# rarimo/ultragroth

Measured on AMD Instinct MI355X. Metric: proofs/s, higher is better.
Workload: dtype u32x9 (29-bit limbs, 254-bit modular integers)

## Files before the change

### ultragroth_amd/csrc/internal.hpp

```cpp
#pragma once
#include <hip/hip_runtime.h>
#include <cstdint>
#include <cstddef>
#include <vector>
#include "ec.hpp"
#include "stream_timer.hpp"

namespace ug {

Fr fr_root_of_unity(int s);
void bitrev_copy(u32* out, const u32* in, int logn, hipStream_t stream);

struct NttFusion {
    const u32* in2 = nullptr; u32* work = nullptr; const u32* fin_a = nullptr; const u32* fin_b = nullptr;
    u64 in2_stride = 0, work_stride = 0, fin_a_stride = 0, fin_b_stride = 0;
};

struct NttPass {
    const u32* in; u32* out; const u32* tw; const u32* post; const u32* post_const; const u32* in2; const u32* fin_a; const u32* fin_b;
    int logn, s0, k, j, gather_bitrev, scatter_bitrev;
    u64 in_stride, out_stride, in2_stride, fin_a_stride, fin_b_stride;
};
constexpr int NTT_MAX_PASSES = 8;

struct NttPlan {
    int logn = -1;
    u32* tw_fwd = nullptr;
    u32* tw_inv = nullptr;
    u32* twist = nullptr;
    u32* ninv = nullptr;
    bool shoup = true;
    void init(int logn, hipStream_t stream);
    void release();
    void transform(u32* out, const u32* in, bool inverse, bool gather_bitrev, bool scatter_bitrev,
                   const u32* post, const u32* post_const, hipStream_t stream, LaunchTimer stats = LaunchTimer(),
                   const struct NttFusion* fuse = nullptr, int vectors = 1, u64 out_stride = 0, u64 in_stride = 0) const;
    int passes(NttPass* list, u32* out, const u32* in, bool inverse, bool gather_bitrev, bool scatter_bitrev,
               const u32* post, const u32* post_const, const struct NttFusion* fuse = nullptr, u64 out_stride = 0, u64 in_stride = 0) const;
    void launch(const NttPass* const* lists, int count, int p, hipStream_t stream, LaunchTimer stats = LaunchTimer(), int vectors = 1) const;
    ~NttPlan() { release(); }
};

uint64_t alloc_epoch();
void alloc_epoch_bump();
template <class T> void epoch_alloc(T*& p, size_t bytes) { alloc_epoch_bump(); if (p) hipFree(p); p = nullptr; UG_HIP(hipMalloc(&p, bytes ? bytes : 4)); }

struct BucketClasses {
    int q_log = 0;
    u32 r0 = 0, cnt = 1;
    u32 specials = 0;
    u32 sp_lo = 0, sp_hi = 0;
    bool on() const { return q_log > 0; }
};
constexpr u32 MSM_MAX_SPECIALS = 64;

struct DigitPlan {
    u64 n; int c, windows; u32 buckets, sentinel; int tables;
    u64 set_map, table_map;
    int q_log; u32 r0, cnt, specials, sp_lo, sp_hi, special_base;
    u32 vec_count, vec_magic; int vec_shift; u32 vec_sets; u64 vec_stride;
};

struct MsmGeometry {
    u64 n = 0;
    int c = 0;
    int windows = 0;
    u32 buckets = 0;
    bool tables = false;
    int stride = 1;
    BucketClasses cls;
    int vectors = 1;
    u64 vec_stride = 0;
    static MsmGeometry choose(u64 n, int force_c = 0);
    static MsmGeometry choose_tables(u64 n, int c, int stride = 1);
    static int table_window(u64 n);
    static int table_count(int c, int stride) { const int w = (255 + c - 1) / c; return (w + stride - 1) / stride; }
    void set_classes(const BucketClasses& k);
    void set_vectors(int v, u64 stride);
    u64 vector_count() const { return n / (u64)vectors; }
    int window_sets() const { return tables ? stride : windows; }
    int class_sets() const { return cls.on() ? (int)cls.cnt : 1; }
    int bucket_windows() const { return window_sets() * class_sets() * vectors; }
    u64 special_buckets() const { return cls.on() ? (u64)window_sets() * cls.specials : 0; }
    u64 total_buckets() const { return (u64)bucket_windows() * buckets + special_buckets(); }
    int result_points() const { return cls.on() ? 2 * bucket_windows() + (cls.specials ? window_sets() : 0) : bucket_windows(); }
    u64 expected_entries() const { return cls.on() ? ((n * (u64)windows) >> cls.q_log) * cls.cnt : n * (u64)windows; }
    DigitPlan digit_plan() const {
        DigitPlan d;
        d.n = n; d.c = c; d.windows = windows; d.buckets = buckets; d.sentinel = (u32)total_buckets(); d.tables = tables ? 1 : 0;
        d.set_map = 0; d.table_map = 0;
        if (tables)
            for (int w = 0; w < windows && w < 16; w++) { d.set_map |= (u64)(w % stride) << (4 * w); d.table_map |= (u64)(w / stride) << (4 * w); }
        d.q_log = cls.q_log; d.r0 = cls.r0; d.cnt = cls.on() ? cls.cnt : 1; d.specials = cls.on() ? cls.specials : 0;
        d.sp_lo = cls.sp_lo; d.sp_hi = cls.sp_hi; d.special_base = (u32)((u64)bucket_windows() * buckets);
        d.vec_count = (u32)vector_count(); d.vec_magic = 0; d.vec_shift = 0; d.vec_sets = (u32)window_sets(); d.vec_stride = vec_stride;
        if (vectors > 1) {
            int l = 0;
            while (((u64)1 << l) < (u64)d.vec_count) l++;
            d.vec_magic = (u32)((((u64)1 << 32) * (((u64)1 << l) - d.vec_count)) / d.vec_count + 1);
            d.vec_shift = l;
        }
        return d;
    }
};
constexpr int MSM_MAX_VECTORS = 16;
constexpr int TABLE_INDEX_BITS = 27;
constexpr int TABLE_MIN_C = 16, TABLE_MAX_C = 24;
double msm_model_cost(u64 n, int c, bool tables, int stride = 1);

struct HeavyBucket { u32 bucket, first_seg, last_seg, pad; };

int radix_plan(int bits, int* shift, int* bins_log);
void digit_pairs(const u32* scalars, const DigitPlan& plan, u32* keys, u32* vals, hipStream_t stream);
struct RadixSorter {
    u32* lookback = nullptr;
    u32* small = nullptr;
    u64 tiles_cap = 0;
    void reserve(u64 n_pairs, int ipt_min);
    void release();
    int sort(const u32* scalars, const MsmGeometry& geo, u32 sentinel, u64 n_pairs, int bits,
             u32* const buf_keys[2], u32* const buf_vals[2], u32* error_flag, hipStream_t stream, u32* n_valid_out = nullptr,
             bool* dropped_out = nullptr);
    ~RadixSorter() { release(); }
};

struct MsmSchedule {
    MsmGeometry geo;
    const u32* keys = nullptr;
    const u32* vals = nullptr;
    const u32* tkeys = nullptr;
    const u32* tvals = nullptr;
    u32* bucket_start = nullptr;
    u32* bucket_count = nullptr;
    u32* small_list = nullptr;
    int log_seg = 0;
    int log_seg_tail = 0;
    u32* heavy_list = nullptr;
    u32 heavy_cap = 0;
    u32* medium_list = nullptr;
    u32* heavy_offsets = nullptr;
    u32* meta = nullptr;
    u32 *keys_a = nullptr, *keys_b = nullptr, *vals_a = nullptr, *vals_b = nullptr;
    void* sort_tmp = nullptr; size_t sort_tmp_bytes = 0;
    RadixSorter sorter;
    u64 capacity_n = 0; u64 capacity_buckets = 0;
    void reserve(const MsmGeometry& g);
    void build(const u32* scalars_dev, const MsmGeometry& g, hipStream_t stream);
    void release();
    ~MsmSchedule() { release(); }
};

struct MsmWorkspace {
    u32* bucket_pts = nullptr;
    u32* chunk_pts = nullptr;
    u32* chunk_pts2 = nullptr;
    u32* slot_pts = nullptr;
    u32* task_pts = nullptr;
    size_t bucket_bytes = 0, chunk_bytes = 0, slot_bytes = 0, task_bytes = 0;
    void reserve(const MsmGeometry& g, bool g2, u64 n_segments, u32 n_heavy_tasks, int sets = 1);
    void release();
    ~MsmWorkspace() { release(); }
};

struct MsmPending {
    bool g2 = false;
    bool empty = true;
    int c = 0, window_sets = 0, class_sets = 1;
    int vectors = 1;
    BucketClasses cls;
    u32* host = nullptr;
};
constexpr int MSM_G2_PT_WORDS = 72;
constexpr size_t MSM_PENDING_WORDS = 128 * 72;
constexpr int MSM_QUEUE_DEPTH = 8;
constexpr int MSM_BATCH_WIDTH = 4;
struct MsmCall {
    struct Product { const u32* bases = nullptr; u64 n_bases = 0; int64_t delta = 0; u32* host = nullptr; };
    int count = 0;
    Product products[MSM_BATCH_WIDTH];
    int group = 0;
};
constexpr int MSM_PHASE_ALL = 0, MSM_PHASE_ACCUMULATE = 1, MSM_PHASE_TAIL = 2;
void msm_enqueue(bool g2, const MsmSchedule& s, MsmWorkspace& ws, const MsmCall& call, hipStream_t stream, LaunchTimer stats, MsmPending* pend,
                 int phase = MSM_PHASE_ALL);
void interleave_points_g1(u32* dst, const u32* src, u64 n, int members, int member, u64 slot0, hipStream_t stream);
G1XYZZ msm_collect_g1(const MsmPending& p, int vector = 0);
G2XYZZ msm_collect_g2(const MsmPending& p, int vector = 0);

void convert_points_g1(u32* pts, u64 n, hipStream_t stream);
void convert_points_g2(u32* pts, u64 n, hipStream_t stream);

void build_window_tables(bool g2, u32* pts, u64 n, int doublings, int tables, hipStream_t stream, u64 first = 0, u64 count = ~(u64)0);

void synth_points(bool g2, u32* out_dev, const u32* gen_record_host, u64 seed, u64 n, hipStream_t stream);

void check_points(bool g2, const u32* pts, u64 n, u64 index0, int level, unsigned long long* fault, hipStream_t stream);
void check_points_mask(bool g2, const u32* pts, u64 n, int level, uint8_t* status, hipStream_t stream);

struct CoefMatrix {
    u64 ncoefs = 0; u32 domain = 0; int logn = 0;
    u32* row_ptr = nullptr;
    u32* sig = nullptr;
    u32* val = nullptr;
    bool build(const uint8_t* raw44_dev, u64 ncoefs, u32 domain, u32 nvars, hipStream_t stream);
    void release();
    ~CoefMatrix() { release(); }
};

void coef_matvec(u32* a_br, u32* b_br, const CoefMatrix& m, const u32* wtns_dev, int mask, hipStream_t stream);
constexpr int MATVEC_VT = 4;
void coef_matvec_vectors(u32* a_br, u32* b_br, u64 out_stride, const CoefMatrix& m, const u32* wtns_dev, u64 wtns_stride, int vectors,
                         hipStream_t stream);
void fr_mul_pointwise(u32* out, const u32* x, const u32* y, u64 n, hipStream_t stream);
void fr_h_final(u32* h, const u32* a, const u32* b, const u32* c, u64 n, hipStream_t stream);
void fr_h_final_vectors(u32* h, u64 h_stride, const u32* a, const u32* b, const u32* c, u64 in_stride, u64 n, int vectors, hipStream_t stream);
void fr_from_mont256(u32* out, const u32* in, u64 n, hipStream_t stream);
void fr_to_mont256(u32* out, const u32* in, u64 n, hipStream_t stream);
void f_op_mont256(int which, int op, u32* out, const u32* a, const u32* b, u64 n, hipStream_t stream);
void gather_elements(u32* out, const u32* src, const u32* index_dev, u64 n, u64 src_n, hipStream_t stream);
void scatter_elements(u32* dst, const u32* index_dev, const u32* values_dev, u64 n, u64 dst_n, hipStream_t stream);
void lookup_table(u32* table_dev, const u32* freq_dev, u64 L, hipStream_t stream);
void apply_lookup(u32* dst, u32* last_scratch, const u32* w_idx, const u32* p_idx, u64 n, const u32* chunks, u64 n_chunks,
                  const u32* table, hipStream_t stream);
struct LookupVec { u64 n, n_chunks, L, w_off, p_off, c_off, f_off, r_off, t_off; };
void lookup_tables_vectors(u32* stage, const LookupVec* vec_dev, int vectors, u64 max_L, hipStream_t stream);
void apply_lookup_vectors(u32* dst, u64 stride, u32* last_scratch, const u32* stage, const LookupVec* vec_dev, int vectors, u64 max_n,
                          hipStream_t stream);


struct R1csDev {
    u32 rows = 0;
    const u32* row_ptr[3] = {nullptr, nullptr, nullptr};
    const u32* sig[3] = {nullptr, nullptr, nullptr};
    const u32* val[3] = {nullptr, nullptr, nullptr};
};
void r1cs_convert_coefs(u32* val, u64 n, hipStream_t stream);
void r1cs_check(const R1csDev& m, const u32* wtns, unsigned long long* words, uint8_t* mask, hipStream_t stream);
void r1cs_row_values(const R1csDev& m, const u32* wtns, u32 k, u32* out24, hipStream_t stream);
void r1cs_match(const R1csDev& m, const CoefMatrix& zk, u32 n_public, const u32* z, unsigned long long* word, hipStream_t stream);

}
```

### ultragroth_amd/csrc/msm.hip

```cpp
#ifdef UG_MEASURE
#include <hipcub/hipcub.hpp>
#endif
#include <algorithm>
#include <atomic>
#include <cstdlib>
#include <cstring>
#include <string>
#include <type_traits>
#include "dev_common.hpp"
#include "internal.hpp"
#include "segmap.hpp"

namespace ug {

namespace {

constexpr int LOG_SEG = 7;
constexpr u32 FIX_MAX = 32;
constexpr u32 MEDIUM_MAX = 4096;
constexpr u32 HEAVY_TASK = 1024;
constexpr int CHUNK = 32;

constexpr int ACC_BLOCK = 256;

// ... 345 lines not shown
    u32 nkey = cur, nval = tvals[tbase];
    int64_t nidx = (int64_t)(nval & IDX_MASK) + delta;
    bool nin = nidx >= 0 && (u64)nidx < n_slots;
    if (nin) Cfg::load_raw(raw, record(nval, nidx, 0));
    for (u32 k = 0; k < cnt; k++) {
        const u32 key = nkey, val = nval;
        const int64_t idx = nidx;
        const bool in = nin;
        const bool more = k + 1 < cnt;
        if (more) {
            nkey = tkeys[tbase + ((u64)(k + 1) << 6)];
            nval = tvals[tbase + ((u64)(k + 1) << 6)];
            nidx = (int64_t)(nval & IDX_MASK) + delta;
            nin = nidx >= 0 && (u64)nidx < n_slots;
        }
        if (key != cur) {
            flush(first_run && start_open, (size_t)2 * t, cur);
            cur = key;
            first_run = false;
        }
        StaticFor<0, K>::up([&](auto m) {
            F x, y;
            const bool valid = in && Cfg::decode_affine(raw, x, y);
            if (m + 1 < K) { if (in) Cfg::load_raw(raw, record(val, idx, m + 1)); }
            else if (more && nin) Cfg::load_raw(raw, record(nval, nidx, 0));
            if (valid && (val >> 31)) y = neg<1>(y);
            if (valid) acc[m] = xyzz_madd(acc[m], x, y);
        });
    }
    const bool end_open = hi < n_valid && keys[hi] == cur;
    if (first_run && start_open) flush(true, (size_t)2 * t, 0);
    else if (end_open) flush(true, (size_t)2 * t + 1, 0);
    else flush(false, 0, cur);
}

template <class Cfg>
__device__ __forceinline__ XYZZ<typename Cfg::F> load_piece(const u32* slot_pts, u32 first, u32 k) {
    size_t slot = k ? (size_t)2 * (first + k) : (size_t)2 * first + 1;
    return Cfg::from_words(slot_pts + slot * Cfg::PT_WORDS, 1);
}

template <class Cfg>
__global__ __launch_bounds__(128) void bucket_fixup_kernel(const u32* __restrict__ small_list, const u32* __restrict__ meta,
                                                           const u32* __restrict__ start, const u32* __restrict__ count, int log_a, int log_b,
                                                           const u32* __restrict__ slot_pts, u32* __restrict__ bucket_pts,
                                                           size_t slot_stride, size_t bucket_stride) {
    u32 t = blockIdx.x * blockDim.x + threadIdx.x;
    if (t >= meta[4]) return;
    slot_pts += blockIdx.y * slot_stride; bucket_pts += blockIdx.y * bucket_stride;
    typedef typename Cfg::F F;
    const u32 b = small_list[t];
    const u32 st = start[b];
    const SegMap map = SegMap::make(meta[1], log_a, log_b);
    const u32 first = map.seg_of(st), last = map.seg_of(st + count[b] - 1);
    const u32 pieces = last - first + 1;
    XYZZ<F> acc = load_piece<Cfg>(slot_pts, first, 0);
    for (u32 k = 1; k < pieces; k++) acc = xyzz_add(acc, load_piece<Cfg>(slot_pts, first, k));
    Cfg::to_words(bucket_pts + (size_t)b * Cfg::PT_WORDS, acc, 1);
}

template <class Cfg>
__device__ __forceinline__ XYZZ<typename Cfg::F> block_reduce(XYZZ<typename Cfg::F> acc, u32* lds) {
    const int tid = threadIdx.x, nth = Cfg::BLOCK;
    for (int stride = nth / 2; stride > 0; stride >>= 1) {
        if (tid >= stride && tid < 2 * stride) Cfg::to_words(lds + (tid - stride), acc, stride);
        __syncthreads();
        if (tid < stride) acc = xyzz_add(acc, Cfg::from_words(lds + tid, stride));
        __syncthreads();
    }
    return acc;
}

template <class Cfg>
__global__ __launch_bounds__(256) void medium_bucket_kernel(const HeavyBucket* mb, const u32* meta, u32 cap, const u32* slot_pts, u32* bucket_pts,
                                                            size_t slot_stride, size_t bucket_stride) {
    typedef typename Cfg::F F;
    slot_pts += blockIdx.y * slot_stride; bucket_pts += blockIdx.y * bucket_stride;
    const u32 lane = threadIdx.x & 63, n_waves = (gridDim.x * blockDim.x) >> 6;
    const u32 n_medium = meta[3] < cap ? meta[3] : cap;
    for (u32 wave = (blockIdx.x * blockDim.x + threadIdx.x) >> 6; wave < n_medium; wave += n_waves) {
        HeavyBucket h = mb[wave];
        u32 pieces = h.last_seg - h.first_seg + 1;
        XYZZ<F> acc = xyzz_inf<F>();
        for (u32 k = lane; k < pieces; k += 64) acc = xyzz_add(acc, load_piece<Cfg>(slot_pts, h.first_seg, k));
        u32 w[Cfg::PT_WORDS];
        for (int off = 32; off > 0; off >>= 1) {
            Cfg::to_words(w, acc, 1);
#pragma unroll
            for (int i = 0; i < Cfg::PT_WORDS; i++) w[i] = __shfl_xor(w[i], off, 64);
            acc = xyzz_add(acc, Cfg::from_words(w, 1));
        }
        if (lane == 0) Cfg::to_words(bucket_pts + (size_t)h.bucket * Cfg::PT_WORDS, acc, 1);
    }
}

__global__ __launch_bounds__(1024) void heavy_plan_kernel(const HeavyBucket* hb, u32 n_heavy_cap, u32* meta, u32* offsets) {
    __shared__ u32 part[1024];
    const u32 n = meta[0] < n_heavy_cap ? meta[0] : n_heavy_cap;
    const u32 per = (n + 1023) / 1024;
    u32 lo = threadIdx.x * per, hi = lo + per < n ? lo + per : n;
    u32 sum = 0;
    for (u32 i = lo; i < hi; i++) sum += (hb[i].last_seg - hb[i].first_seg + 1 + HEAVY_TASK - 1) / HEAVY_TASK;
    part[threadIdx.x] = sum;
    __syncthreads();
    if (threadIdx.x == 0) {
        u32 run = 0;
        for (int i = 0; i < 1024; i++) { u32 v = part[i]; part[i] = run; run += v; }
        meta[2] = run;
        offsets[n] = run;
    }
    __syncthreads();
    u32 run = part[threadIdx.x];
    for (u32 i = lo; i < hi; i++) {
        offsets[i] = run;
        run += (hb[i].last_seg - hb[i].first_seg + 1 + HEAVY_TASK - 1) / HEAVY_TASK;
    }
}

template <class Cfg>
__global__ __launch_bounds__(Cfg::BLOCK) void heavy_partial_kernel(const HeavyBucket* hb, const u32* offsets, const u32* meta, u32 cap,
                                                                   const u32* slot_pts, u32* task_pts, size_t slot_stride, size_t task_stride) {
    __shared__ u32 lds[Cfg::PT_WORDS * Cfg::BLOCK / 2];
    typedef typename Cfg::F F;
    slot_pts += blockIdx.y * slot_stride; task_pts += blockIdx.y * task_stride;
    const u32 task = blockIdx.x;
    const u32 n_heavy = meta[0] < cap ? meta[0] : cap;
    if (task >= meta[2]) return;
    u32 lo = 0, hi = n_heavy;
    while (hi - lo > 1) { u32 mid = (lo + hi) >> 1; if (offsets[mid] <= task) lo = mid; else hi = mid; }
    HeavyBucket h = hb[lo];
    u32 pieces = h.last_seg - h.first_seg + 1;
    u32 p0 = (task - offsets[lo]) * HEAVY_TASK, p1 = p0 + HEAVY_TASK < pieces ? p0 + HEAVY_TASK : pieces;
    XYZZ<F> acc = xyzz_inf<F>();
    for (u32 k = p0 + threadIdx.x; k < p1; k += Cfg::BLOCK) acc = xyzz_add(acc, load_piece<Cfg>(slot_pts, h.first_seg, k));
    acc = block_reduce<Cfg>(acc, lds);
    if (threadIdx.x == 0) Cfg::to_words(task_pts + (size_t)task * Cfg::PT_WORDS, acc, 1);
}

template <class Cfg>
__global__ __launch_bounds__(Cfg::BLOCK) void heavy_final_kernel(const HeavyBucket* hb, const u32* offsets, const u32* meta, u32 cap,
                                                                 const u32* task_pts, u32* bucket_pts, size_t task_stride, size_t bucket_stride) {
    __shared__ u32 lds[Cfg::PT_WORDS * Cfg::BLOCK / 2];
    typedef typename Cfg::F F;
    task_pts += blockIdx.y * task_stride; bucket_pts += blockIdx.y * bucket_stride;
    if (blockIdx.x >= (meta[0] < cap ? meta[0] : cap)) return;
    HeavyBucket h = hb[blockIdx.x];
    u32 t0 = offsets[blockIdx.x], t1 = offsets[blockIdx.x + 1];
    XYZZ<F> acc = xyzz_inf<F>();
    for (u32 k = t0 + threadIdx.x; k < t1; k += Cfg::BLOCK) acc = xyzz_add(acc, Cfg::from_words(task_pts + (size_t)k * Cfg::PT_WORDS, 1));
    acc = block_reduce<Cfg>(acc, lds);
    if (threadIdx.x == 0) Cfg::to_words(bucket_pts + (size_t)h.bucket * Cfg::PT_WORDS, acc, 1);
}

template <class Cfg>
__global__ __launch_bounds__(128) void bucket_chunk_reduce_kernel(const u32* buckets, const u32* count, u32 per_window, int chunk,
                                                                  u32 nchunks_total, int scalar_bits, u32* out, u32 windows, u32* out0,
                                                                  size_t product_buckets) {
    u32 t = blockIdx.x * blockDim.x + threadIdx.x;
    if (t >= nchunks_total) return;
    typedef typename Cfg::F F;
    u32 chunks_per_window = per_window / chunk;
    u32 w = t / chunks_per_window, j = t % chunks_per_window;
    const size_t b0 = (size_t)(w / windows) * product_buckets + (size_t)(w % windows) * per_window + (size_t)j * chunk;
    const size_t c0 = (size_t)(w % windows) * per_window + (size_t)j * chunk;
    const u32* base = buckets + b0 * Cfg::PT_WORDS;
    XYZZ<F> run = xyzz_inf<F>(), acc = xyzz_inf<F>();
    for (int k = chunk - 1; k >= 0; k--) {
        if (count[c0 + k]) run = xyzz_add(run, Cfg::from_words(base + (size_t)k * Cfg::PT_WORDS, 1));
        acc = xyzz_add(acc, run);
    }
    u32 off = j * (u32)chunk;
    if (off) acc = xyzz_add(acc, xyzz_mul_scalar(run, &off, scalar_bits));
    Cfg::to_words(out + (size_t)t * Cfg::PT_WORDS, acc, 1);
    if (out0) Cfg::to_words(out0 + (size_t)t * Cfg::PT_WORDS, run, 1);
}
template <class Cfg>
__global__ __launch_bounds__(64) void special_sum_kernel(const u32* bucket_pts, const u32* count, u32 special_base, u32 S, size_t bucket_stride,
                                                         u32* out, u32 window_sets) {
    typedef typename Cfg::F F;
    const u32 w = blockIdx.x, q = blockIdx.y, lane = threadIdx.x;
    XYZZ<F> x = xyzz_inf<F>();
    const u32 id = special_base + w * S + lane;
    if (lane < S && count[id]) x = Cfg::from_words(bucket_pts + (size_t)q * bucket_stride + (size_t)id * Cfg::PT_WORDS, 1);
    XYZZ<F> acc = xyzz_inf<F>();
    const u32 k = lane + 1;
    for (int i = 6; i >= 0; i--) {
        acc = xyzz_dbl(acc);
        if ((k >> i) & 1) acc = xyzz_add(acc, x);
    }
    u32 v[Cfg::PT_WORDS];
    for (int off = 32; off > 0; off >>= 1) {
        Cfg::to_words(v, acc, 1);
#pragma unroll
        for (int i = 0; i < Cfg::PT_WORDS; i++) v[i] = __shfl_xor(v[i], off, 64);
        acc = xyzz_add(acc, Cfg::from_words(v, 1));
    }
    if (lane == 0) Cfg::to_words(out + ((size_t)q * window_sets + w) * Cfg::PT_WORDS, acc, 1);
}
template <class Cfg>
__global__ __launch_bounds__(128) void ec_sum_groups_kernel(const u32* in, u32* out, u32 n_out, int group) {
    u32 t = blockIdx.x * blockDim.x + threadIdx.x;
    if (t >= n_out) return;
    typedef typename Cfg::F F;
    XYZZ<F> acc = Cfg::from_words(in + (size_t)t * group * Cfg::PT_WORDS, 1);
    for (int g = 1; g < group; g++) acc = xyzz_add(acc, Cfg::from_words(in + ((size_t)t * group + g) * Cfg::PT_WORDS, 1));
    Cfg::to_words(out + (size_t)t * Cfg::PT_WORDS, acc, 1);
}

template <class Cfg>
__global__ __launch_bounds__(256) void ec_sum_wave_kernel(const u32* in, u32* out, u32 n_out, int group) {
    typedef typename Cfg::F F;
    const u32 wave = (blockIdx.x * blockDim.x + threadIdx.x) >> 6, lane = threadIdx.x & 63;
    if (wave >= n_out) return;
    XYZZ<F> acc = xyzz_inf<F>();
    for (int g = (int)lane; g < group; g += 64) acc = xyzz_add(acc, Cfg::from_words(in + ((size_t)wave * group + g) * Cfg::PT_WORDS, 1));
    u32 w[Cfg::PT_WORDS];
    for (int off = 32; off > 0; off >>= 1) {
        Cfg::to_words(w, acc, 1);
#pragma unroll
        for (int i = 0; i < Cfg::PT_WORDS; i++) w[i] = __shfl_xor(w[i], off, 64);
        acc = xyzz_add(acc, Cfg::from_words(w, 1));
    }
    if (lane == 0) Cfg::to_words(out + (size_t)wave * Cfg::PT_WORDS, acc, 1);
}

__global__ void convert_coords_kernel(u32* pts, u64 n_coords_groups, int coords_per_point) {
    u64 i = (u64)blockIdx.x * blockDim.x + threadIdx.x;
    if (i >= n_coords_groups) return;
    u32* p = pts + i * 8 * coords_per_point;
    u32 o = 0;
    for (int k = 0; k < 8 * coords_per_point; k++) o |= p[k];
    if (o == 0) return;
    for (int k = 0; k < coords_per_point; k++) {
        u32 w[8];
        load8(w, p + 8 * k);
        Fq v = cond_sub_q(from_mont256<FqParams>(w));
        pack256(w, v);
        store8(p + 8 * k, w);
    }
}

__global__ void interleave_records_kernel(u32* __restrict__ dst, const u32* __restrict__ src, u64 n, int members, int member, u64 slot0) {
    const u64 g = (u64)blockIdx.x * blockDim.x + threadIdx.x;
    if (g >= n * 4) return;
    const u64 i = g >> 2, part = g & 3;
    reinterpret_cast<uint4*>(dst + ((slot0 + i) * (u64)members + (u64)member) * 16)[part] = reinterpret_cast<const uint4*>(src + i * 16)[part];
}

template <class Cfg, int K>
__global__ __launch_bounds__(128) void window_tables_kernel(u32* pts, u64 n_all, int c, int tables, u64 first, u64 end) {
    typedef typename Cfg::F F;
    const u64 i0 = first + ((u64)blockIdx.x * blockDim.x + threadIdx.x) * K;
    const u64 n = end;
    if (i0 >= n) return;
    F x[K], y[K];
    bool live[K];
    StaticFor<0, K>::up([&](auto k) { live[k] = i0 + k < n && Cfg::load_affine(pts + (i0 + k) * Cfg::AFF_WORDS, x[k], y[k]); });
    for (int j = 1; j < tables; j++) {
        XYZZ<F> p[K];
        StaticFor<0, K>::up([&](auto k) { p[k] = live[k] ? xyzz_dbl_affine(x[k], y[k]) : xyzz_inf<F>(); });
        for (int d = 1; d < c; d++)
            StaticFor<0, K>::up([&](auto k) { p[k] = xyzz_dbl(p[k]); });
        F pre[K];
        F run = field_one((F*)0);
        StaticFor<0, K>::up([&](auto k) {
            pre[k] = run;
            if (live[k]) run = mulk<8>(run, p[k].zzz);
        });
        F irun = inv(run);
        StaticFor<0, K>::down([&](auto k) {
            if (i0 + k >= n) return;
            u32* o = pts + ((u64)j * n_all + i0 + k) * Cfg::AFF_WORDS;
            if (live[k]) {
                F izzz = mulk<8>(irun, pre[k]);
                irun = mulk<8>(irun, p[k].zzz);
                F iz = mulk<8>(izzz, p[k].zz);
                F izz = sqrk<8>(iz);
                x[k] = canon(mulk<8>(p[k].x, izz));
                y[k] = canon(mulk<8>(p[k].y, izzz));
                Cfg::store_affine_packed(o, x[k], y[k]);
            } else {
                for (int w = 0; w < Cfg::AFF_WORDS; w++) o[w] = 0;
            }
        });
    }
}

template <class Cfg>
__global__ __launch_bounds__(128) void synth_points_kernel(const u32* table, u64 seed, u64 n, u32* out) {
    u64 i = (u64)blockIdx.x * blockDim.x + threadIdx.x;
    if (i >= n) return;
    typedef typename Cfg::F F;
    u64 k = seed + i;
    XYZZ<F> acc = xyzz_inf<F>();
    for (int j = 0; j < 64; j++) {
        if (!((k >> j) & 1)) continue;
        F x, y;
        Cfg::load_affine(table + (size_t)j * Cfg::AFF_WORDS, x, y);
        acc = xyzz_madd(acc, x, y);
    }
    u32* o = out + i * Cfg::AFF_WORDS;
    if (is_inf(acc)) { for (int w = 0; w < Cfg::AFF_WORDS; w++) o[w] = 0; return; }
    F ax, ay;
    xyzz_to_affine(ax, ay, acc);
    Cfg::store_affine_mont256(o, ax, ay);
}

int reduce_chunk(const MsmGeometry& g, int sets = 1, bool g2 = false) {
    static const int g2_log = getenv("UG_REDUCE_G2_LOG") ? atoi(getenv("UG_REDUCE_G2_LOG")) : 16;
    static const int g1_log = getenv("UG_REDUCE_G1_LOG") ? atoi(getenv("UG_REDUCE_G1_LOG")) : 0;
    const int g1_auto = (u64)sets * g.bucket_windows() * g.buckets < ((u64)1 << 21) ? 16 : 17;
    const u64 lanes = (u64)1 << (g2 ? g2_log : (g1_log ? g1_log : g1_auto));
    int chunk = g.buckets < (u32)CHUNK ? (int)g.buckets : CHUNK;
    while (chunk > 8 && (u64)sets * g.bucket_windows() * (g.buckets / chunk) < lanes) chunk >>= 1;
    return chunk;
}

template <class T> void dev_free(T*& p) { if (p) { alloc_epoch_bump(); hipFree(p); } p = nullptr; }
std::atomic<uint64_t> g_alloc_epoch{1};

}

uint64_t alloc_epoch() { return g_alloc_epoch.load(std::memory_order_acquire); }
void alloc_epoch_bump() { g_alloc_epoch.fetch_add(1, std::memory_order_acq_rel); }

namespace {
int segment_log(u64 total_entries) {
    static const int lanes_log = getenv("UG_SEG_LANES_LOG") ? atoi(getenv("UG_SEG_LANES_LOG")) : 20;
    int log_seg = 5;
    while (log_seg < LOG_SEG && (total_entries >> (log_seg + 1)) >= ((u64)1 << lanes_log)) log_seg++;
    return log_seg;
}
double msm_cost(u64 n, int c, bool tables, int stride = 1) {
    const int windows = (255 + c - 1) / c;
    const double entries = (double)windows * (double)n, buckets = (double)((u64)1 << (c - 1));
    const double sets = tables ? (double)stride : (double)windows;
    const double per_bucket = entries / (sets * buckets);
    const double over = per_bucket / (double)((u64)1 << segment_log((u64)entries)) - 1.0;
    return entries * (1.0 + (over > 0 ? 0.04 * over : 0.0)) + 4.0 * buckets * sets;
}
}

double msm_model_cost(u64 n, int c, bool tables, int stride) { return msm_cost(n, c, tables, stride); }

MsmGeometry MsmGeometry::choose(u64 n, int force_c) {
    MsmGeometry g;
    g.n = n;
    int c = force_c;
    if (!c) {
        static const int env_c = getenv("UG_MSM_C") ? atoi(getenv("UG_MSM_C")) : 0;
        c = env_c;
    }
    if (!c) {
        double best = 0;
        for (int k = 6; k <= 22; k++) {
            double cost = msm_cost(n, k, false);
            if (!c || cost < best) { best = cost; c = k; }
        }
    }
    if (c < 2) c = 2;
    if (c > 22) c = 22;
    g.c = c;
    g.windows = (255 + c - 1) / c;
    g.buckets = 1u << (c - 1);
    return g;
}

int MsmGeometry::table_window(u64 n) {
    if (const char* e = getenv("UG_TABLE_C")) {
        int v = atoi(e);
        if (v >= TABLE_MIN_C && v <= TABLE_MAX_C) return v;
    }
    int c = 0;
    double best = 0;
    for (int k = TABLE_MIN_C; k <= TABLE_MAX_C; k++) {
        double cost = msm_cost(n, k, true);
        if (!c || cost < best) { best = cost; c = k; }
    }
    return c;
}
MsmGeometry MsmGeometry::choose_tables(u64 n, int c, int stride) {
    if (c < TABLE_MIN_C || c > TABLE_MAX_C) throw std::invalid_argument("msm: table window width outside [16, 24]");
    MsmGeometry g;
    g.n = n; g.c = c; g.tables = true;
    g.windows = (255 + c - 1) / c;
    g.buckets = 1u << (c - 1);
    if (stride < 1 || stride > g.windows)
        throw std::invalid_argument("msm: table stride " + std::to_string(stride) + " outside [1, " + std::to_string(g.windows) + "]");
    g.stride = stride;
    return g;
}

void MsmGeometry::set_classes(const BucketClasses& k) {
    cls = BucketClasses();
    if (!k.on()) return;
    if (k.q_log > 8) throw std::invalid_argument("msm: more than 256 bucket classes");
    if (tables && stride > 1) throw std::invalid_argument("msm: bucket classes need one bucket set per product (table stride 1)");
    const u32 Q = 1u << k.q_log;
    if (k.cnt < 1 || k.r0 + k.cnt > Q) throw std::invalid_argument("msm: bucket residues outside [0, 2^q_log)");
    if (k.specials > MSM_MAX_SPECIALS) throw std::invalid_argument("msm: more than 64 special buckets");
    if (k.sp_lo > k.sp_hi || k.sp_hi > n) throw std::invalid_argument("msm: special-bucket scalar range outside the schedule");
    if (c - 1 < k.q_log + 3 || ((u64)1 << (c - 1)) < k.specials) throw std::invalid_argument("msm: window too narrow for this many bucket classes");
    cls = k;
    buckets = 1u << (c - 1 - k.q_log);
    if ((size_t)result_points() * 72 > MSM_PENDING_WORDS - 1) throw std::invalid_argument("msm: too many bucket sets for one result block");
}

static_assert(G2Cfg::PT_WORDS == MSM_G2_PT_WORDS, "internal.hpp: MSM_G2_PT_WORDS");
void MsmGeometry::set_vectors(int v, u64 stride) {
    vectors = 1; vec_stride = 0;
    if (v == 1) return;
    if (v < 1 || v > MSM_MAX_VECTORS) throw std::invalid_argument("msm: vectors outside [1, " + std::to_string(MSM_MAX_VECTORS) + "]");
    if (cls.on()) throw std::invalid_argument("msm: bucket classes cannot be combined with several scalar vectors");
    if (stride < n) throw std::invalid_argument("msm: vector stride below the scalars per vector");
    if (n == 0) throw std::invalid_argument("msm: several vectors of no scalars");
    const u64 total = n * (u64)v;
    if (total * (u64)windows > ((u64)1 << 30)) throw std::invalid_argument("msm: vectors * n * windows exceeds 2^30 entries");
    if ((u64)window_sets() * (u64)v * buckets >= ((u64)1 << 31)) throw std::invalid_argument("msm: more than 2^31 buckets over all vectors");
    if ((size_t)window_sets() * (size_t)v * MSM_G2_PT_WORDS > MSM_PENDING_WORDS - 1)
        throw std::invalid_argument("msm: too many bucket sets over all vectors for one result block");
    vectors = v; vec_stride = stride; n = total;
}

void MsmSchedule::reserve(const MsmGeometry& g) {
    u64 total = g.n * g.windows;
    if (total > capacity_n) {
        u64 padded = total + ((u64)64 << LOG_SEG);
        epoch_alloc(keys_a, padded * 4); epoch_alloc(keys_b, padded * 4);
        epoch_alloc(vals_a, padded * 4); epoch_alloc(vals_b, padded * 4);
        dev_free(sort_tmp); sort_tmp_bytes = 0;
        sorter.reserve(total, 12);
        capacity_n = total;
    }
    if (g.total_buckets() > capacity_buckets) {
        epoch_alloc(bucket_start, g.total_buckets() * 4);
        epoch_alloc(bucket_count, g.total_buckets() * 4);
        epoch_alloc(small_list, g.total_buckets() * 4);
        capacity_buckets = g.total_buckets();
    }
    u64 hcap = (total >> 5) / (FIX_MAX - 1) + 2;
    if (hcap > heavy_cap) {
        epoch_alloc(heavy_list, 4 * hcap * 4); epoch_alloc(medium_list, 4 * hcap * 4); epoch_alloc(heavy_offsets, (hcap + 1) * 4);
        heavy_cap = (u32)hcap;
    }
    if (!meta) epoch_alloc(meta, 32);
}

void MsmSchedule::build(const u32* scalars_dev, const MsmGeometry& g, hipStream_t stream) {
    if (g.n * (u64)g.windows > ((u64)1 << 30)) throw std::invalid_argument("msm: n * windows exceeds 2^30 entries");
    if (g.vector_count() > ((u64)1 << TABLE_INDEX_BITS)) throw std::invalid_argument("msm: more than 2^27 scalars in one schedule");
    geo = g;
    reserve(g);
    log_seg = segment_log(g.expected_entries());
    static const bool taper = !(getenv("UG_SEG_TAPER") && atoi(getenv("UG_SEG_TAPER")) == 0);
    log_seg_tail = (taper && log_seg == LOG_SEG && (g.expected_entries() >> log_seg) >= ((u64)1 << 16)) ? log_seg - 2 : log_seg;
    if (g.n == 0) return;
    u64 total = g.n * g.windows;
    u32 nb = (u32)g.total_buckets();
    u32 sentinel = nb;
    int end_bit = 1;
    while (((u64)1 << end_bit) <= sentinel) end_bit++;
    UG_HIP(hipMemsetAsync(meta, 0, 32, stream));
#ifdef UG_MEASURE
    static const bool use_cub = getenv("UG_SORT") && !strcmp(getenv("UG_SORT"), "cub");
#else
    constexpr bool use_cub = false;
#endif
    const bool pairs_first = use_cub || g.windows > 16;
    bool dropped = false;
    if (pairs_first) digit_pairs(scalars_dev, g.digit_plan(), keys_a, vals_a, stream);
#ifdef UG_MEASURE
    if (use_cub) {
        hipcub::DoubleBuffer<u32> dk(keys_a, keys_b), dv(vals_a, vals_b);
        if (!sort_tmp_bytes) {
            size_t need = 0;
            UG_HIP(hipcub::DeviceRadixSort::SortPairs(nullptr, need, dk, dv, (int)total, 0, 32));
            epoch_alloc(sort_tmp, need); sort_tmp_bytes = need;
        }
        size_t tmp = sort_tmp_bytes;
        UG_HIP(hipcub::DeviceRadixSort::SortPairs(sort_tmp, tmp, dk, dv, (int)total, 0, end_bit, stream));
        keys = dk.Current();
        vals = dv.Current();
    } else
#endif
    {
        u32* const bk[2] = {keys_a, keys_b};
        u32* const bv[2] = {vals_a, vals_b};
        const int at = sorter.sort(pairs_first ? nullptr : scalars_dev, g, sentinel, total, end_bit, bk, bv, meta + 7, stream, meta + 1, &dropped);
        keys = bk[at];
        vals = bv[at];
    }
    UG_HIP(hipMemsetAsync(bucket_start, 0, (size_t)nb * 4, stream));
    UG_HIP(hipMemsetAsync(bucket_count, 0, (size_t)nb * 4, stream));
    hipLaunchKernelGGL(bucket_bounds_kernel, dim3((unsigned)((total + 1023) / 1024)), dim3(256), 0, stream,
                       keys, total, sentinel, bucket_start, bucket_count, meta, dropped ? 1 : 0);
    UG_KERNEL_CHECK();
    hipLaunchKernelGGL(bucket_counts_kernel, dim3((nb + 1023) / 1024), dim3(1024), 0, stream, bucket_start, bucket_count, nb,
                       log_seg, log_seg_tail, meta, heavy_list, medium_list, heavy_cap, small_list);
    UG_KERNEL_CHECK();
    hipLaunchKernelGGL(heavy_plan_kernel, dim3(1), dim3(1024), 0, stream, (const HeavyBucket*)heavy_list, heavy_cap, meta, heavy_offsets);
    UG_KERNEL_CHECK();
    u64 n_tiles = (SegMap::max_segments(total, log_seg, log_seg_tail) + 63) / 64;
    u32* tk = (keys == keys_a) ? keys_b : keys_a;
    u32* tv = (vals == vals_a) ? vals_b : vals_a;
    {
        size_t lds = (size_t)2 * 64 * (((size_t)1 << log_seg) + 1) * 4;
        hipLaunchKernelGGL(transpose_entries_kernel, dim3((unsigned)n_tiles), dim3(1024), lds, stream,
                           keys, vals, meta, sentinel, log_seg, log_seg_tail, tk, tv);
        UG_KERNEL_CHECK();
    }
    tkeys = tk; tvals = tv;
}

void MsmSchedule::release() {
    dev_free(keys_a); dev_free(keys_b); dev_free(vals_a); dev_free(vals_b); dev_free(sort_tmp);
    dev_free(bucket_start); dev_free(bucket_count); dev_free(small_list); dev_free(heavy_list); dev_free(medium_list); dev_free(heavy_offsets); dev_free(meta);
    sorter.release();
    capacity_n = capacity_buckets = 0; sort_tmp_bytes = 0; vals = nullptr; keys = nullptr; heavy_cap = 0;
}

void MsmWorkspace::reserve(const MsmGeometry& g, bool g2, u64 n_segments, u32 n_heavy_tasks, int sets) {
    size_t ptw = (size_t)(g2 ? G2Cfg::PT_WORDS : G1Cfg::PT_WORDS) * (size_t)sets;
    size_t need = (size_t)g.total_buckets() * ptw * 4;
    if (need > bucket_bytes) { epoch_alloc(bucket_pts, need); bucket_bytes = need; }
    const int chunk = reduce_chunk(g, sets, g2);
    size_t cneed = ((size_t)(g.cls.on() ? 2 : 1) * g.bucket_windows() * (g.buckets / chunk) + (size_t)g.window_sets()) * ptw * 4;
    if (cneed > chunk_bytes) { epoch_alloc(chunk_pts, cneed); epoch_alloc(chunk_pts2, cneed); chunk_bytes = cneed; }
    size_t sneed = (size_t)n_segments * 2 * ptw * 4;
    if (sneed > slot_bytes) { epoch_alloc(slot_pts, sneed); slot_bytes = sneed; }
    size_t tneed = (size_t)n_heavy_tasks * ptw * 4;
    if (tneed > task_bytes) { epoch_alloc(task_pts, tneed); task_bytes = tneed; }
}
void MsmWorkspace::release() {
    dev_free(bucket_pts); dev_free(chunk_pts); dev_free(chunk_pts2); dev_free(slot_pts); dev_free(task_pts);
    bucket_bytes = chunk_bytes = slot_bytes = task_bytes = 0;
}

namespace {
template <class Cfg>
void msm_enqueue_multi(const MsmSchedule& s, MsmWorkspace& ws, const MsmCall& call, hipStream_t stream, LaunchTimer stats, MsmPending* pend, int phase) {
    const int count = call.count, group = call.group;
    const MsmCall::Product* const p = call.products;
    const bool do_acc = phase != MSM_PHASE_TAIL, do_tail = phase != MSM_PHASE_ACCUMULATE;
    typedef typename Cfg::F F;
    const MsmGeometry& g = s.geo;
    if (count < 1 || count > MSM_BATCH_WIDTH) throw std::logic_error("msm: batch size");
    int live[MSM_BATCH_WIDTH], k = 0;
    for (int j = 0; j < count; j++) {
        pend[j] = MsmPending();
        pend[j].g2 = Cfg::PT_WORDS == G2Cfg::PT_WORDS;
        pend[j].c = g.c; pend[j].window_sets = g.window_sets(); pend[j].class_sets = g.class_sets(); pend[j].cls = g.cls; pend[j].vectors = g.vectors;
        pend[j].host = p[j].host;
        if (g.n == 0 || p[group ? 0 : j].n_bases == 0) continue;
        if ((size_t)g.result_points() * Cfg::PT_WORDS > MSM_PENDING_WORDS - 1) throw std::logic_error("msm: result block too large");
        pend[j].empty = false;
        live[k++] = j;
    }
    if (!k) return;
    const u64 total = g.n * g.windows;
    const u64 nseg = SegMap::max_segments(total, s.log_seg, s.log_seg_tail);
    const u32 heavy_max = (u32)std::min<u64>(s.heavy_cap, nseg / MEDIUM_MAX + 1);
    const u32 tasks_max = (u32)((nseg + heavy_max) / HEAVY_TASK + heavy_max + 1);
    const u32 medium_max = (u32)std::min<u64>(s.heavy_cap, nseg / (FIX_MAX - 1) + 1);
    if (do_acc) ws.reserve(g, Cfg::PT_WORDS == G2Cfg::PT_WORDS, nseg, tasks_max, k);
    const size_t bucket_stride = (size_t)g.total_buckets() * Cfg::PT_WORDS, slot_stride = (size_t)nseg * 2 * Cfg::PT_WORDS,
                 task_stride = (size_t)tasks_max * Cfg::PT_WORDS;
    if constexpr (Cfg::PT_WORDS == G1Cfg::PT_WORDS) {
        if (group && do_acc) {
#ifdef UG_MEASURE
            const char* fold = getenv("UG_GROUP_FOLD_LOG");
            const u32 fold_mask = fold && *fold ? ((1u << atoi(fold)) - 1) : ~0u;
#define UG_FOLD_ARG , fold_mask
#else
#define UG_FOLD_ARG
#endif
            StreamTimer::Scope timed = stats.time(stream, g.n * g.windows * (u64)group);
            if (nseg) {
                const dim3 grid((unsigned)((nseg + 255) / 256)), block(256);
#define UG_GROUP_LAUNCH(K_) hipLaunchKernelGGL((segment_accumulate_group_kernel<K_>), grid, block, 0, stream, p[0].bases, p[0].n_bases, \
                                                   p[0].delta, s.keys, s.tkeys, s.tvals, s.meta, s.log_seg, s.log_seg_tail, ws.bucket_pts, ws.slot_pts,   \
                                                   bucket_stride, slot_stride UG_FOLD_ARG)
                if (group == 3) UG_GROUP_LAUNCH(3);
                else if (group == 2) UG_GROUP_LAUNCH(2);
                else throw std::logic_error("msm: group size");
#undef UG_GROUP_LAUNCH
#undef UG_FOLD_ARG
                UG_KERNEL_CHECK();
            }
            timed.stop();
        }
    } else if (group) throw std::logic_error("msm: groups are G1 only");
    for (int q = 0; q < (group || !do_acc ? 0 : k); q++) {
        const int j = live[q];
        StreamTimer::Scope timed = stats.time(stream, g.n * g.windows);
        if (nseg) {
            hipLaunchKernelGGL(segment_accumulate_kernel<Cfg>, dim3((unsigned)((nseg + ACC_BLOCK - 1) / ACC_BLOCK)), dim3(ACC_BLOCK), 0, stream,
                               p[j].bases, p[j].n_bases, p[j].delta, s.keys, s.tkeys, s.tvals, s.meta, s.log_seg, s.log_seg_tail,
                               ws.bucket_pts + q * bucket_stride, ws.slot_pts + q * slot_stride);
            UG_KERNEL_CHECK();
        }
        timed.stop();
    }
    if (!do_tail) return;
    if (nseg > 1) {
        const u64 small_max = std::min<u64>(g.total_buckets(), nseg);
        hipLaunchKernelGGL(bucket_fixup_kernel<Cfg>, dim3((unsigned)((small_max + 127) / 128), k), dim3(128), 0, stream,
                           s.small_list, s.meta, s.bucket_start, s.bucket_count, s.log_seg, s.log_seg_tail, ws.slot_pts, ws.bucket_pts,
                           slot_stride, bucket_stride);
        UG_KERNEL_CHECK();
        if (nseg > FIX_MAX) {
            hipLaunchKernelGGL(medium_bucket_kernel<Cfg>, dim3(std::min<u32>((medium_max + 3) / 4, 2048), k), dim3(256), 0, stream,
                               (const HeavyBucket*)s.medium_list, s.meta, medium_max, ws.slot_pts, ws.bucket_pts, slot_stride, bucket_stride);
            UG_KERNEL_CHECK();
        }
        if (nseg > MEDIUM_MAX) {
            hipLaunchKernelGGL(heavy_partial_kernel<Cfg>, dim3(tasks_max, k), dim3(Cfg::BLOCK), 0, stream,
                               (const HeavyBucket*)s.heavy_list, s.heavy_offsets, s.meta, heavy_max, ws.slot_pts, ws.task_pts,
                               slot_stride, task_stride);
            UG_KERNEL_CHECK();
            hipLaunchKernelGGL(heavy_final_kernel<Cfg>, dim3(heavy_max, k), dim3(Cfg::BLOCK), 0, stream,
                               (const HeavyBucket*)s.heavy_list, s.heavy_offsets, s.meta, heavy_max, ws.task_pts, ws.bucket_pts,
                               task_stride, bucket_stride);
            UG_KERNEL_CHECK();
        }
    }
    int chunk = reduce_chunk(g, k, Cfg::PT_WORDS == G2Cfg::PT_WORDS);
    const int windows = g.bucket_windows();
    const int bw = windows * k;
    const bool classes = g.cls.on();
    u32 cpw = g.buckets / chunk;
    u32 nchunks = cpw * bw;
    hipLaunchKernelGGL(bucket_chunk_reduce_kernel<Cfg>, dim3((nchunks + 127) / 128), dim3(128), 0, stream,
                       ws.bucket_pts, s.bucket_count, g.buckets, chunk, nchunks, g.c, ws.chunk_pts, (u32)windows,
                       classes ? ws.chunk_pts + (size_t)nchunks * Cfg::PT_WORDS : (u32*)nullptr, (size_t)g.total_buckets());
    UG_KERNEL_CHECK();
    const int tree_sets = classes ? 2 * bw : bw;
    u32* cur = ws.chunk_pts; u32* nxt = ws.chunk_pts2;
    while (cpw > 1) {
        if ((u64)(cpw / 16) * tree_sets >= 8192) {
            const int group = 16;
            u32 n_out = (cpw / group) * tree_sets;
            hipLaunchKernelGGL(ec_sum_groups_kernel<Cfg>, dim3((n_out + 127) / 128), dim3(128), 0, stream, cur, nxt, n_out, group);
            cpw /= group;
        } else {
            const int group = cpw >= 256 ? 256 : (int)cpw;
            u32 n_out = (cpw / group) * tree_sets;
            hipLaunchKernelGGL(ec_sum_wave_kernel<Cfg>, dim3((n_out + 3) / 4), dim3(256), 0, stream, cur, nxt, n_out, group);
            cpw /= group;
        }
        UG_KERNEL_CHECK();
        std::swap(cur, nxt);
    }
    const int wsets = g.window_sets();
    const bool specials = classes && g.cls.specials;
    if (specials) {
        hipLaunchKernelGGL(special_sum_kernel<Cfg>, dim3((unsigned)wsets, (unsigned)k), dim3(64), 0, stream, ws.bucket_pts, s.bucket_count,
                           (u32)((u64)windows * g.buckets), g.cls.specials, bucket_stride, cur + (size_t)tree_sets * Cfg::PT_WORDS, (u32)wsets);
        UG_KERNEL_CHECK();
    }
    for (int q = 0; q < k; q++) {
        u32* host = p[live[q]].host;
        const size_t set_words = (size_t)windows * Cfg::PT_WORDS;
        UG_HIP(hipMemcpyAsync(host, cur + (size_t)q * set_words, set_words * 4, hipMemcpyDeviceToHost, stream));
        if (classes) UG_HIP(hipMemcpyAsync(host + set_words, cur + ((size_t)bw + (size_t)q * windows) * Cfg::PT_WORDS, set_words * 4, hipMemcpyDeviceToHost, stream));
        if (specials) UG_HIP(hipMemcpyAsync(host + 2 * set_words, cur + ((size_t)tree_sets + (size_t)q * wsets) * Cfg::PT_WORDS,
                                            (size_t)wsets * Cfg::PT_WORDS * 4, hipMemcpyDeviceToHost, stream));
        UG_HIP(hipMemcpyAsync(host + MSM_PENDING_WORDS - 1, s.meta + 7, 4, hipMemcpyDeviceToHost, stream));
    }
}

template <class Cfg>
XYZZ<typename Cfg::F> msm_collect(const MsmPending& p, int vector = 0) {
    typedef typename Cfg::F F;
    XYZZ<F> acc = xyzz_inf<F>();
    if (p.empty) return acc;
    if (p.host[MSM_PENDING_WORDS - 1]) throw std::runtime_error("msm: the schedule's sort gave up waiting for a tile (look-back timeout)");
    if (vector < 0 || vector >= p.vectors) throw std::logic_error("msm: vector index");
    const int sets = p.window_sets * p.class_sets;
    const u32* block = p.host + (size_t)vector * sets * Cfg::PT_WORDS;
    auto point = [&](int idx) { return Cfg::from_words(block + (size_t)idx * Cfg::PT_WORDS, 1); };
    for (int w = p.window_sets - 1; w >= 0; w--) {
        for (int k = 0; k < p.c; k++) acc = xyzz_dbl(acc);
        if (!p.cls.on()) { acc = xyzz_add(acc, point(w)); continue; }
        const int cnt = p.class_sets;
        XYZZ<F> s1 = xyzz_inf<F>(), s0_all = xyzz_inf<F>(), run = xyzz_inf<F>(), steps = xyzz_inf<F>();
        for (int j = 0; j < cnt; j++) {
            s1 = xyzz_add(s1, point(w * cnt + j));
            const XYZZ<F> s0 = point(sets + w * cnt + j);
            s0_all = xyzz_add(s0_all, s0);
            if (j + 1 < cnt) { run = xyzz_add(run, s0); steps = xyzz_add(steps, run); }
        }
        for (int k = 0; k < p.cls.q_log; k++) s1 = xyzz_dbl(s1);
        const u32 m_last = (1u << p.cls.q_log) - p.cls.r0 - (u32)cnt;
        XYZZ<F> minus = xyzz_add(steps, xyzz_mul_scalar(s0_all, &m_last, 9));
        XYZZ<F> wsum = xyzz_add(s1, xyzz_neg(minus));
        if (p.cls.specials) wsum = xyzz_add(wsum, point(2 * sets + w));
        acc = xyzz_add(acc, wsum);
    }
    return acc;
}
}

void msm_enqueue(bool g2, const MsmSchedule& s, MsmWorkspace& ws, const MsmCall& call, hipStream_t stream, LaunchTimer stats, MsmPending* pend,
                 int phase) {
    if (call.group && (call.group < 2 || call.group > 3 || call.count != call.group)) throw std::invalid_argument("msm: a base group has 2 or 3 members");
    if (!g2) msm_enqueue_multi<G1Cfg>(s, ws, call, stream, stats, pend, phase);
    else msm_enqueue_multi<G2Cfg>(s, ws, call, stream, stats, pend, phase);
}
G1XYZZ msm_collect_g1(const MsmPending& p, int vector) { return msm_collect<G1Cfg>(p, vector); }
G2XYZZ msm_collect_g2(const MsmPending& p, int vector) { return msm_collect<G2Cfg>(p, vector); }

namespace {
template <class Cfg>
void synth_points_run(u32* out_dev, const u32* gen_record_host, u64 seed, u64 n, hipStream_t stream) {
    typedef typename Cfg::F F;
    std::vector<u32> table((size_t)64 * Cfg::AFF_WORDS);
    std::vector<u32> gen(gen_record_host, gen_record_host + Cfg::AFF_WORDS);
    XYZZ<F> p;
    {
        F x, y;
        const int nc = Cfg::AFF_WORDS / 8;
        Fq c[4];
        for (int k = 0; k < nc; k++) c[k] = from_mont256<FqParams>(gen.data() + 8 * k);
        if (nc == 2) { memcpy(&x, &c[0], sizeof(Fq)); memcpy(&y, &c[1], sizeof(Fq)); }
        else { memcpy(&x, &c[0], 2 * sizeof(Fq)); memcpy(&y, &c[2], 2 * sizeof(Fq)); }
        p = xyzz_from_affine(x, y);
    }
    for (int j = 0; j < 64; j++) {
        F ax, ay;
        xyzz_to_affine(ax, ay, p);
        Cfg::store_affine_packed(table.data() + (size_t)j * Cfg::AFF_WORDS, ax, ay);
        p = xyzz_dbl(p);
    }
    u32* d_table = nullptr;
    UG_HIP(hipMalloc(&d_table, table.size() * 4));
    UG_HIP(hipMemcpyAsync(d_table, table.data(), table.size() * 4, hipMemcpyHostToDevice, stream));
    hipLaunchKernelGGL(synth_points_kernel<Cfg>, dim3((unsigned)((n + 127) / 128)), dim3(128), 0, stream, d_table, seed, n, out_dev);
    UG_KERNEL_CHECK();
    UG_HIP(hipStreamSynchronize(stream));
    hipFree(d_table);
}
}

void synth_points(bool g2, u32* out_dev, const u32* gen_record_host, u64 seed, u64 n, hipStream_t stream) {
    if (!n) return;
    if (g2) synth_points_run<G2Cfg>(out_dev, gen_record_host, seed, n, stream);
    else synth_points_run<G1Cfg>(out_dev, gen_record_host, seed, n, stream);
}

void build_window_tables(bool g2, u32* pts, u64 n, int doublings, int tables, hipStream_t stream, u64 first, u64 count) {
    if (!n || tables < 2) return;
    if (first > n) first = n;
    const u64 end = count > n - first ? n : first + count, m = end - first;
    if (!m) return;
    if (g2) {
        hipLaunchKernelGGL((window_tables_kernel<G2Cfg, 2>), dim3((unsigned)(((m + 1) / 2 + 127) / 128)), dim3(128), 0, stream, pts, n, doublings, tables, first, end);
    } else {
        hipLaunchKernelGGL((window_tables_kernel<G1Cfg, 4>), dim3((unsigned)(((m + 3) / 4 + 127) / 128)), dim3(128), 0, stream, pts, n, doublings, tables, first, end);
    }
    UG_KERNEL_CHECK();
}

void interleave_points_g1(u32* dst, const u32* src, u64 n, int members, int member, u64 slot0, hipStream_t stream) {
    if (!n) return;
    hipLaunchKernelGGL(interleave_records_kernel, dim3((unsigned)((n * 4 + 255) / 256)), dim3(256), 0, stream, dst, src, n, members, member, slot0);
    UG_KERNEL_CHECK();
}
void convert_points_g1(u32* pts, u64 n, hipStream_t stream) {
    if (!n) return;
    hipLaunchKernelGGL(convert_coords_kernel, dim3((unsigned)((n + 255) / 256)), dim3(256), 0, stream, pts, n, 2);
    UG_KERNEL_CHECK();
}
void convert_points_g2(u32* pts, u64 n, hipStream_t stream) {
    if (!n) return;
    hipLaunchKernelGGL(convert_coords_kernel, dim3((unsigned)((n + 255) / 256)), dim3(256), 0, stream, pts, n, 4);
    UG_KERNEL_CHECK();
}

}
```

Baseline: 7.808.

## Reduce MSM bucket windows hierarchically with per-chunk running sums and wave-level combining

Replaces the bucket-window reduction for G1 without bucket classes with a multi-level scheme. Each chunk now emits both its weighted sum and its running sum, and a wave-level kernel merges chunk results using doublings by chunk size and cross-lane shuffles. This avoids the old path, which scaled each chunk result by its offset and then summed them with separate tree kernels. It also reuses the bucket buffer as scratch so the second chunk buffer is skipped, and sets the G1 lane target to a fixed 2^17 in place of the auto heuristic. The cost is a complex instruction-sequenced kernel with extra point doublings and shuffles of full points.

```diff
diff --git a/ultragroth_amd/csrc/internal.hpp b/ultragroth_amd/csrc/internal.hpp
--- a/ultragroth_amd/csrc/internal.hpp
+++ b/ultragroth_amd/csrc/internal.hpp
@@ -156,7 +156,7 @@
     u32* chunk_pts2 = nullptr;
     u32* slot_pts = nullptr;
     u32* task_pts = nullptr;
-    size_t bucket_bytes = 0, chunk_bytes = 0, slot_bytes = 0, task_bytes = 0;
+    size_t bucket_bytes = 0, chunk_bytes = 0, chunk2_bytes = 0, slot_bytes = 0, task_bytes = 0;
     void reserve(const MsmGeometry& g, bool g2, u64 n_segments, u32 n_heavy_tasks, int sets = 1);
     void release();
     ~MsmWorkspace() { release(); }
diff --git a/ultragroth_amd/csrc/msm.hip b/ultragroth_amd/csrc/msm.hip
--- a/ultragroth_amd/csrc/msm.hip
+++ b/ultragroth_amd/csrc/msm.hip
@@ -521,6 +521,96 @@
     if (threadIdx.x == 0) Cfg::to_words(bucket_pts + (size_t)h.bucket * Cfg::PT_WORDS, acc, 1);
 }
 
+
+template <class Cfg>
+__global__ __launch_bounds__(128) void bucket_chunk_sums_kernel(const u32* buckets, const u32* count, u32 per_window, int chunk,
+                                                                u32 nchunks_total, u32* out_t, u32* out_r, u32 windows,
+                                                                size_t product_buckets) {
+    u32 t = blockIdx.x * blockDim.x + threadIdx.x;
+    if (t >= nchunks_total) return;
+    typedef typename Cfg::F F;
+    u32 chunks_per_window = per_window / chunk;
+    u32 w = t / chunks_per_window, j = t % chunks_per_window;
+    const size_t b0 = (size_t)(w / windows) * product_buckets + (size_t)(w % windows) * per_window + (size_t)j * chunk;
+    const size_t c0 = (size_t)(w % windows) * per_window + (size_t)j * chunk;
+    const u32* base = buckets + b0 * Cfg::PT_WORDS;
+    XYZZ<F> run = xyzz_inf<F>(), acc = xyzz_inf<F>();
+    for (int k = chunk - 1; k >= 0; k--) {
+        if (count[c0 + k]) run = xyzz_add(run, Cfg::from_words(base + (size_t)k * Cfg::PT_WORDS, 1));
+        acc = xyzz_add(acc, run);
+    }
+    Cfg::to_words(out_t + (size_t)t * Cfg::PT_WORDS, acc, 1);
+    Cfg::to_words(out_r + (size_t)t * Cfg::PT_WORDS, run, 1);
+}
+
+template <class Cfg>
+__device__ __forceinline__ XYZZ<typename Cfg::F> lane_exchange(const XYZZ<typename Cfg::F>& p, u32 from) {
+    u32 v[Cfg::PT_WORDS];
+    Cfg::to_words(v, p, 1);
+#pragma unroll
+    for (int i = 0; i < Cfg::PT_WORDS; i++) v[i] = __shfl(v[i], (int)from, 64);
+    return Cfg::from_words(v, 1);
+}
+
+template <class Cfg>
+__global__ __launch_bounds__(256) void bucket_level_kernel(const u32* in_t, const u32* in_r, u32 m, int q, int log_q, int log_in, int steps,
+                                                           u32 m_out, u32 n_waves, u32* out_t, u32* out_r) {
+    typedef typename Cfg::F F;
+    const u32 wave = (blockIdx.x * blockDim.x + threadIdx.x) >> 6, lane = threadIdx.x & 63;
+    if (wave >= n_waves) return;
+    const u32 set = wave / m_out, e0 = ((wave % m_out) * 64 + lane) * (u32)q;
+    const size_t first = (size_t)set * m;
+    const int p0 = 2 * q, p1 = p0 + 2 * log_in, p2 = p1 + q, p3 = p2 + steps, p4 = p3 + (out_r ? 6 + log_q : 0), p5 = p4 + 1,
+              p6 = p5 + log_q, p7 = p6 + 1, p8 = p7 + steps;
+    enum { LOAD, OTHER, LANE };
+    XYZZ<F> run = xyzz_inf<F>(), w = xyzz_inf<F>();
+    for (int i = 0; i < p8; i++) {
+        bool dbl = false, on_w = false, pred = true;
+        int operand = OTHER;
+        const u32* src = nullptr;
+        u32 from = lane;
+        if (i < p0) {
+            const u32 t = (u32)(q - 1 - (i >> 1));
+            if (i & 1) { on_w = true; pred = t > 0; }
+            else { operand = LOAD; src = in_r + (first + e0 + t) * Cfg::PT_WORDS; pred = e0 + t < m; }
+        } else if (i < p1) {
+            dbl = true; on_w = !((i - p0) & 1);
+        } else if (i < p2) {
+            const u32 t = (u32)(i - p1);
+            on_w = true; operand = LOAD; src = in_t + (first + e0 + t) * Cfg::PT_WORDS; pred = e0 + t < m;
+        } else if (i < p3) {
+            operand = LANE; from = lane + (1u << (i - p2)); pred = from < 64;
+        } else if (i < p4) {
+            dbl = true; pred = lane == 0;
+        } else if (i < p5) {
+            if (lane == 0) {
+                if (out_r) Cfg::to_words(out_r + (size_t)wave * Cfg::PT_WORDS, run, 1);
+                run = xyzz_inf<F>();
+            }
+            continue;
+        } else if (i < p6) {
+            dbl = true;
+        } else if (i < p7) {
+            on_w = true;
+        } else {
+            on_w = true; operand = LANE; from = lane ^ ((1u << steps) >> (1 + i - p7));
+        }
+        if (on_w) { const XYZZ<F> x = run; run = w; w = x; }
+        if (dbl) {
+            if (pred) run = xyzz_dbl(run);
+        } else {
+            XYZZ<F> b = xyzz_inf<F>();
+            if (operand == LANE) b = lane_exchange<Cfg>(run, from & 63);
+            if (operand == OTHER) b = w;
+            if (operand == LOAD && pred) b = Cfg::from_words(src, 1);
+            if (!pred) b = xyzz_inf<F>();
+            run = xyzz_add(run, b);
+        }
+        if (on_w) { const XYZZ<F> x = run; run = w; w = x; }
+    }
+    if (lane == 0) Cfg::to_words(out_t + (size_t)wave * Cfg::PT_WORDS, w, 1);
+}
+
 template <class Cfg>
 __global__ __launch_bounds__(128) void bucket_chunk_reduce_kernel(const u32* buckets, const u32* count, u32 per_window, int chunk,
                                                                   u32 nchunks_total, int scalar_bits, u32* out, u32 windows, u32* out0,
@@ -677,12 +767,21 @@
 
 int reduce_chunk(const MsmGeometry& g, int sets = 1, bool g2 = false) {
     static const int g2_log = getenv("UG_REDUCE_G2_LOG") ? atoi(getenv("UG_REDUCE_G2_LOG")) : 16;
-    static const int g1_log = getenv("UG_REDUCE_G1_LOG") ? atoi(getenv("UG_REDUCE_G1_LOG")) : 0;
-    const int g1_auto = (u64)sets * g.bucket_windows() * g.buckets < ((u64)1 << 21) ? 16 : 17;
-    const u64 lanes = (u64)1 << (g2 ? g2_log : (g1_log ? g1_log : g1_auto));
+    static const int g1_log = getenv("UG_REDUCE_G1_LOG") ? atoi(getenv("UG_REDUCE_G1_LOG")) : 17;
+    const u64 lanes = (u64)1 << (g2 ? g2_log : g1_log);
     int chunk = g.buckets < (u32)CHUNK ? (int)g.buckets : CHUNK;
     while (chunk > 8 && (u64)sets * g.bucket_windows() * (g.buckets / chunk) < lanes) chunk >>= 1;
     return chunk;
+}
+bool reduce_in_levels(const MsmGeometry& g, bool g2) {
+    static const int which = getenv("UG_REDUCE_LEVELS") ? atoi(getenv("UG_REDUCE_LEVELS")) : 1;
+    return !g.cls.on() && which > (g2 ? 1 : 0);
+}
+int level_lanes_log(u32 m, u32 sets) {
+    static const int waves_log = getenv("UG_LEVEL_WAVES_LOG") ? atoi(getenv("UG_LEVEL_WAVES_LOG")) : 10;
+    int log_q = 0;
+    while (((u64)64 << log_q) < m && (u64)sets * ((m + ((u64)64 << log_q) - 1) / ((u64)64 << log_q)) > ((u64)1 << waves_log)) log_q++;
+    return log_q;
 }
 
 template <class T> void dev_free(T*& p) { if (p) { alloc_epoch_bump(); hipFree(p); } p = nullptr; }
@@ -893,8 +992,9 @@
     size_t need = (size_t)g.total_buckets() * ptw * 4;
     if (need > bucket_bytes) { epoch_alloc(bucket_pts, need); bucket_bytes = need; }
     const int chunk = reduce_chunk(g, sets, g2);
-    size_t cneed = ((size_t)(g.cls.on() ? 2 : 1) * g.bucket_windows() * (g.buckets / chunk) + (size_t)g.window_sets()) * ptw * 4;
-    if (cneed > chunk_bytes) { epoch_alloc(chunk_pts, cneed); epoch_alloc(chunk_pts2, cneed); chunk_bytes = cneed; }
+    size_t cneed = ((size_t)2 * g.bucket_windows() * (g.buckets / chunk) + (size_t)g.window_sets()) * ptw * 4;
+    if (cneed > chunk_bytes) { epoch_alloc(chunk_pts, cneed); chunk_bytes = cneed; }
+    if (!reduce_in_levels(g, g2) && cneed > chunk2_bytes) { epoch_alloc(chunk_pts2, cneed); chunk2_bytes = cneed; }
     size_t sneed = (size_t)n_segments * 2 * ptw * 4;
     if (sneed > slot_bytes) { epoch_alloc(slot_pts, sneed); slot_bytes = sneed; }
     size_t tneed = (size_t)n_heavy_tasks * ptw * 4;
@@ -902,7 +1002,7 @@
 }
 void MsmWorkspace::release() {
     dev_free(bucket_pts); dev_free(chunk_pts); dev_free(chunk_pts2); dev_free(slot_pts); dev_free(task_pts);
-    bucket_bytes = chunk_bytes = slot_bytes = task_bytes = 0;
+    bucket_bytes = chunk_bytes = chunk2_bytes = slot_bytes = task_bytes = 0;
 }
 
 namespace {
@@ -999,12 +1099,35 @@
     const bool classes = g.cls.on();
     u32 cpw = g.buckets / chunk;
     u32 nchunks = cpw * bw;
-    hipLaunchKernelGGL(bucket_chunk_reduce_kernel<Cfg>, dim3((nchunks + 127) / 128), dim3(128), 0, stream,
-                       ws.bucket_pts, s.bucket_count, g.buckets, chunk, nchunks, g.c, ws.chunk_pts, (u32)windows,
-                       classes ? ws.chunk_pts + (size_t)nchunks * Cfg::PT_WORDS : (u32*)nullptr, (size_t)g.total_buckets());
-    UG_KERNEL_CHECK();
     const int tree_sets = classes ? 2 * bw : bw;
     u32* cur = ws.chunk_pts; u32* nxt = ws.chunk_pts2;
+    if (reduce_in_levels(g, Cfg::PT_WORDS == G2Cfg::PT_WORDS)) {
+        u32* in_t = ws.chunk_pts; u32* in_r = in_t + (size_t)nchunks * Cfg::PT_WORDS;
+        hipLaunchKernelGGL(bucket_chunk_sums_kernel<Cfg>, dim3((nchunks + 127) / 128), dim3(128), 0, stream,
+                           ws.bucket_pts, s.bucket_count, g.buckets, chunk, nchunks, in_t, in_r, (u32)windows, (size_t)g.total_buckets());
+        UG_KERNEL_CHECK();
+        u32* spare[2] = {ws.bucket_pts, ws.chunk_pts};
+        int log_chunk = 0;
+        while ((1 << log_chunk) < chunk) log_chunk++;
+        for (int level = 0; cpw > 1; level++) {
+            const int log_q = level_lanes_log(cpw, (u32)bw), q = 1 << log_q;
+            const u32 m_out = (cpw + 64 * (u32)q - 1) / (64 * (u32)q), n_waves = m_out * (u32)bw;
+            int steps = 6;
+            if (m_out == 1) for (steps = 0; ((u32)q << steps) < cpw; steps++) {}
+            u32* out_t = spare[level & 1];
+            u32* out_r = m_out == 1 ? (u32*)nullptr : out_t + (size_t)n_waves * Cfg::PT_WORDS;
+            hipLaunchKernelGGL(bucket_level_kernel<Cfg>, dim3((n_waves + 3) / 4), dim3(256), 0, stream, in_t, in_r, cpw, q, log_q,
+                               level ? 0 : log_chunk, steps, m_out, n_waves, out_t, out_r);
+            UG_KERNEL_CHECK();
+            in_t = out_t; in_r = out_r; cpw = m_out;
+        }
+        cur = in_t;
+    } else {
+        hipLaunchKernelGGL(bucket_chunk_reduce_kernel<Cfg>, dim3((nchunks + 127) / 128), dim3(128), 0, stream,
+                           ws.bucket_pts, s.bucket_count, g.buckets, chunk, nchunks, g.c, ws.chunk_pts, (u32)windows,
+                           classes ? ws.chunk_pts + (size_t)nchunks * Cfg::PT_WORDS : (u32*)nullptr, (size_t)g.total_buckets());
+        UG_KERNEL_CHECK();
+    }
     while (cpw > 1) {
         if ((u64)(cpw / 16) * tree_sets >= 8192) {
             const int group = 16;
```

Result: no change. 7.806 (median of 2 runs) (-0.0%).
